# Renmusxd/PyIsingMonteCarlo

Hardware: AMD Instinct MI355X
Metric: spin-flip attempts/s (whole node), 4096^2 2D Ising (higher is better)
Workload: dtype u32; 1 GPU; c2: 4096x4096 periodic Ising J=-1 beta=0.4407, 256 replicas/GPU, checkerboard Metropolis, bit-packed spins, Philox4x32-10; replicas_per_gpu=256, parallelism=replicas x1

## Files before the change

pyisingmontecarlo_amd/csrc/lattice_kernels.hpp:

```cpp
#pragma once
#include "lattice_types.hpp"
#include "philox.hpp"
#include <type_traits>

namespace isingmc {

__device__ __forceinline__ uint32_t sel4(uint4 v, uint32_t i)
{
    return i == 0 ? v.x : i == 1 ? v.y : i == 2 ? v.z : v.w;
}

struct QuadNbr {
    uint32_t up[4], dn[4], ce[4], si[4];
};

template <bool UNI>
__device__ __forceinline__ void thread_to_quad(const LatGeom &g, uint32_t gid, uint32_t &Q, uint32_t &y,
                                               uint32_t &xw)
{
    if constexpr (UNI) {
        const uint32_t cl = uint32_t(g.cols_log2), col = gid & ((1u << cl) - 1);
        if (cl >= 6) {
            y = gid >> cl;
        } else {
// ... 75 lines not shown
        const uint32_t sw = mem.oth1(row_base(y) + sx);
        own[0] = o4.x; own[1] = o4.y; own[2] = o4.z; own[3] = o4.w;
        n.ce[0] = c4.x; n.ce[1] = c4.y; n.ce[2] = c4.z; n.ce[3] = c4.w;
        n.up[0] = u4.x; n.up[1] = u4.y; n.up[2] = u4.z; n.up[3] = u4.w;
        n.dn[0] = d4.x; n.dn[1] = d4.y; n.dn[2] = d4.z; n.dn[3] = d4.w;
        n.si[0] = sw;
        side_words(n, odd);
#pragma unroll
        for (int q = 0; q < 4; q++) widx[q] = w0 + q;
    } else {
#pragma unroll
        for (int q = 0; q < 4; q++) {
            const uint32_t w = 4 * Q + q;
            const uint32_t yy = w / g.wpr, xx = w - yy * g.wpr;
            const uint32_t yu = (yy == 0 ? g.H : yy) - 1, yd = (yy + 1 == g.H) ? 0 : yy + 1;
            const uint32_t row = yy * g.wpr;
            widx[q] = w;
            own[q] = mem.own1(w);
            n.ce[q] = mem.oth1(w);
            n.up[q] = mem.oth1(yu * g.wpr + xx);
            n.dn[q] = mem.oth1(yd * g.wpr + xx);
            if ((yy + colour) & 1) {
                const uint32_t nxt = mem.oth1(row + (xx + 1 == g.wpr ? 0 : xx + 1));
                n.si[q] = (n.ce[q] >> 1) | (nxt << 31);
            } else {
                const uint32_t prv = mem.oth1(row + (xx == 0 ? g.wpr : xx) - 1);
                n.si[q] = (n.ce[q] << 1) | (prv >> 31);
            }
        }
    }
}

template <bool PMJ>
__device__ __forceinline__ void bond_masks(const uint32_t own, const QuadNbr &n, int q,
                                           const uint32_t *__restrict__ jneg, uint32_t wpp,
                                           uint32_t widx, uint32_t jneg_uniform, uint32_t &a0,
                                           uint32_t &a1, uint32_t &a2, uint32_t &a3)
{
    if constexpr (PMJ) {
        a0 = own ^ n.up[q] ^ jneg[widx];
        a1 = own ^ n.dn[q] ^ jneg[wpp + widx];
        a2 = own ^ n.ce[q] ^ jneg[2 * wpp + widx];
        a3 = own ^ n.si[q] ^ jneg[3 * wpp + widx];
    } else {
        const uint32_t o = own ^ jneg_uniform;
        a0 = o ^ n.up[q];
        a1 = o ^ n.dn[q];
        a2 = o ^ n.ce[q];
        a3 = o ^ n.si[q];
    }
}

struct QuadState {
    uint32_t eq3[4], eq4[4], lt[4], und[4];
};

struct ThrBits {
    uint32_t hi3, hi4;
    uint32_t lo3, lo4;
    bool all3, all4;
    bool any_all;
};

__device__ __forceinline__ ThrBits thr_bits(const LatThr thr)
{
    ThrBits b;
    const uint32_t h3 = __builtin_amdgcn_readfirstlane(uint32_t(thr.T3 >> 32));
    const uint32_t h4 = __builtin_amdgcn_readfirstlane(uint32_t(thr.T4 >> 32));
    b.all3 = (h3 >> N_PLANES) != 0;
    b.all4 = (h4 >> N_PLANES) != 0;
    b.any_all = ((h3 | h4) >> N_PLANES) != 0;
    b.hi3 = h3 & ((1u << N_PLANES) - 1);
    b.hi4 = h4 & ((1u << N_PLANES) - 1);
    b.lo3 = uint32_t(thr.T3);
    b.lo4 = uint32_t(thr.T4);
    return b;
}

struct QuadSigns {
    uint32_t w[4][4];
};

template <bool PMJ>
__device__ __forceinline__ void load_signs(const uint32_t *__restrict__ jn, const LatGeom &g, const uint32_t Q, QuadSigns &js)
{
    if constexpr (PMJ) {
#pragma unroll
        for (int d = 0; d < 4; d++) {
            const uint4 v = *reinterpret_cast<const uint4 *>(jn + size_t(d) * g.wpp + 4 * size_t(Q));
            js.w[0][d] = v.x; js.w[1][d] = v.y; js.w[2][d] = v.z; js.w[3][d] = v.w;
        }
    }
}

__device__ __forceinline__ void class_masks(const uint32_t s01, const uint32_t c01, const uint32_t s23, const uint32_t c23,
                                            uint32_t &eq3, uint32_t &eq4)
{
    eq4 = c01 & c23;
    eq3 = __builtin_amdgcn_bitop3_b32(c01, s23, c23 & s01, 0xEA);
    asm("" : "+v"(eq3), "+v"(eq4));
}

template <bool PMJ>
__device__ __forceinline__ void quad_classes(const uint32_t own[4], const QuadNbr &n, const ThrBits &tb, const QuadSigns &js,
                                             const uint32_t jneg_uniform, QuadState &st)
{
    if constexpr (PMJ) {
#pragma unroll
        for (int q = 0; q < 4; q++) {
            const uint32_t a0 = own[q] ^ n.up[q] ^ js.w[q][0];
            const uint32_t a1 = own[q] ^ n.dn[q] ^ js.w[q][1];
            const uint32_t a2 = own[q] ^ n.ce[q] ^ js.w[q][2];
            const uint32_t a3 = own[q] ^ n.si[q] ^ js.w[q][3];
            class_masks(a0 ^ a1, a0 & a1, a2 ^ a3, a2 & a3, st.eq3[q], st.eq4[q]);
        }
    } else {
        uint32_t c01[4], c23[4];
        if (jneg_uniform) {
#pragma unroll
            for (int q = 0; q < 4; q++) {
                c01[q] = __builtin_amdgcn_bitop3_b32(own[q], n.up[q], n.dn[q], 0x81);
                c23[q] = __builtin_amdgcn_bitop3_b32(own[q], n.ce[q], n.si[q], 0x81);
            }
        } else {
#pragma unroll
            for (int q = 0; q < 4; q++) {
                c01[q] = __builtin_amdgcn_bitop3_b32(own[q], n.up[q], n.dn[q], 0x18);
                c23[q] = __builtin_amdgcn_bitop3_b32(own[q], n.ce[q], n.si[q], 0x18);
            }
        }
#pragma unroll
        for (int q = 0; q < 4; q++) class_masks(n.up[q] ^ n.dn[q], c01[q], n.ce[q] ^ n.si[q], c23[q], st.eq3[q], st.eq4[q]);
    }
    if (tb.any_all) {
#pragma unroll
        for (int q = 0; q < 4; q++) {
            if (tb.all3) st.eq3[q] = 0;
            if (tb.all4) st.eq4[q] = 0;
        }
    }
#pragma unroll
    for (int q = 0; q < 4; q++) {
        st.lt[q] = 0;
        st.und[q] = st.eq3[q] | st.eq4[q];
    }
}

__device__ __forceinline__ void plane_step(QuadState &st, const uint32_t rr[4], const int p, const ThrBits &tb)
{
    const auto step = [&](int q, uint32_t tbw) {
        st.lt[q] = __builtin_amdgcn_bitop3_b32(rr[q], tbw, st.lt[q], 0x8E);
        st.und[q] = __builtin_amdgcn_bitop3_b32(st.und[q], rr[q], tbw, 0x90);
    };
    const uint32_t sel = __builtin_amdgcn_readfirstlane(((tb.hi3 >> (N_PLANES - 1 - p)) & 1u) | (((tb.hi4 >> (N_PLANES - 1 - p)) & 1u) << 1));
    if (sel == 3) {
#pragma unroll
        for (int q = 0; q < 4; q++) step(q, st.eq3[q] | st.eq4[q]);
    } else if (sel == 1) {
#pragma unroll
        for (int q = 0; q < 4; q++) step(q, st.eq3[q]);
    } else if (sel == 2) {
#pragma unroll
        for (int q = 0; q < 4; q++) step(q, st.eq4[q]);
    } else {
#pragma unroll
        for (int q = 0; q < 4; q++) {
            st.lt[q] &= ~rr[q];
            st.und[q] &= ~rr[q];
        }
    }
}

template <int NQ>
__device__ __forceinline__ void quad_planes(QuadState (&st)[NQ], const uint32_t (&Q)[NQ], const uint32_t colour, const uint64_t t,
                                            const uint2 key, const PhiloxVKeys &vk, const ThrBits &tb)
{
    const uint32_t c0 = uint32_t(t);
#pragma unroll
    for (int p = N_PLANES - 1; p >= 0; p--) {
        uint32_t rr[NQ][4];
#pragma unroll
        for (int j = 0; j < NQ; j++) {
            const uint4 rnd = philox4x32_10(make_uint4(c0, Q[j], DOM_LAT_SWEEP, ctr2(t, colour, p)), key, vk);
            rr[j][0] = rnd.x; rr[j][1] = rnd.y; rr[j][2] = rnd.z; rr[j][3] = rnd.w;
        }
        auto step = [&](int j, int q, uint32_t tbw) {
            st[j].lt[q] = __builtin_amdgcn_bitop3_b32(rr[j][q], tbw, st[j].lt[q], 0x8E);
            st[j].und[q] = __builtin_amdgcn_bitop3_b32(st[j].und[q], rr[j][q], tbw, 0x90);
        };
        const uint32_t sel = __builtin_amdgcn_readfirstlane(((tb.hi3 >> (N_PLANES - 1 - p)) & 1u) | (((tb.hi4 >> (N_PLANES - 1 - p)) & 1u) << 1));
        if (sel == 3) {
#pragma unroll
            for (int j = 0; j < NQ; j++)
#pragma unroll
                for (int q = 0; q < 4; q++) step(j, q, st[j].eq3[q] | st[j].eq4[q]);
        } else if (sel == 1) {
#pragma unroll
            for (int j = 0; j < NQ; j++)
#pragma unroll
                for (int q = 0; q < 4; q++) step(j, q, st[j].eq3[q]);
        } else if (sel == 2) {
#pragma unroll
            for (int j = 0; j < NQ; j++)
#pragma unroll
                for (int q = 0; q < 4; q++) step(j, q, st[j].eq4[q]);
        } else {
#pragma unroll
            for (int j = 0; j < NQ; j++)
#pragma unroll
                for (int q = 0; q < 4; q++) {
                    st[j].lt[q] &= ~rr[j][q];
                    st[j].und[q] &= ~rr[j][q];
                }
        }
    }
}

struct QuadRandom {
    uint32_t rr[N_PLANES][4];
    uint4 tie;
};

__device__ __forceinline__ void quad_random(QuadRandom &R, const uint32_t Q, const uint32_t colour, const uint64_t t, const uint2 key,
                                            const PhiloxVKeys &vk)
{
    const uint32_t c0 = uint32_t(t);
#pragma unroll
    for (int p = 0; p < N_PLANES; p++) {
        const uint4 rnd = philox4x32_10(make_uint4(c0, Q, DOM_LAT_SWEEP, ctr2(t, colour, p)), key, vk);
        R.rr[p][0] = rnd.x; R.rr[p][1] = rnd.y; R.rr[p][2] = rnd.z; R.rr[p][3] = rnd.w;
    }
    R.tie = philox4x32_10(make_uint4(c0, Q, DOM_LAT_SWEEP, ctr2(t, colour, N_PLANES)), key, vk);
}

__device__ __forceinline__ void quad_ties(const QuadState &st, const uint32_t Q, const uint32_t colour, const uint64_t t,
                                          const uint2 key, const PhiloxVKeys &vk, const ThrBits &tb, uint32_t acc[4],
                                          const uint4 *first_call = nullptr)
{
    const uint32_t c0 = uint32_t(t), c1 = Q;
#pragma unroll
    for (int q = 0; q < 4; q++) acc[q] = __builtin_amdgcn_bitop3_b32(st.eq3[q], st.eq4[q], st.lt[q], 0xAB);
#ifdef ISINGMC_TIMING_ONLY_NO_TIES
    if (false) {
#else
    if (st.und[0] | st.und[1] | st.und[2] | st.und[3]) {
#endif
        const uint4 rnd = first_call ? *first_call : philox4x32_10(make_uint4(c0, c1, DOM_LAT_SWEEP, ctr2(t, colour, N_PLANES)), key, vk);
#ifdef ISINGMC_TIMING_ONLY_NO_TIE_LOOPS
        {
            const uint32_t rr4[4] = {rnd.x, rnd.y, rnd.z, rnd.w};
#pragma unroll
            for (int q = 0; q < 4; q++) acc[q] |= st.und[q] & (0u - uint32_t(rr4[q] < ((st.und[q] & st.eq4[q]) ? tb.lo4 : tb.lo3)));
            return;
        }
#endif
        const uint32_t n_ties = __popc(st.und[0]) + __popc(st.und[1]) + __popc(st.und[2]) + __popc(st.und[3]);
        if (n_ties <= 4) {
            uint32_t r0 = rnd.x, r1 = rnd.y, r2 = rnd.z, r3 = rnd.w;
            uint32_t lo3v, lo4v;
            asm volatile("v_mov_b32 %0, %1" : "=v"(lo3v) : "s"(tb.lo3));
            asm volatile("v_mov_b32 %0, %1" : "=v"(lo4v) : "s"(tb.lo4));
#pragma unroll
            for (int q = 0; q < 4; q++) {
                uint32_t m = st.und[q];
                while (m) {
                    const uint32_t bit = m & (0u - m);
                    m ^= bit;
                    const uint32_t lo = (bit & st.eq4[q]) ? lo4v : lo3v;
                    if (r0 < lo) acc[q] |= bit;
                    r0 = r1; r1 = r2; r2 = r3;
                }
            }
        } else {
            uint32_t nres = 0;
            uint4 w = rnd;
#pragma unroll
            for (int q = 0; q < 4; q++) {
                uint32_t m = st.und[q];
                while (m) {
                    const uint32_t b = __ffs(m) - 1;
                    m &= m - 1;
                    if (nres != 0 && (nres & 3u) == 0)
                        w = philox4x32_10(make_uint4(c0, c1, DOM_LAT_SWEEP, ctr2(t, colour, N_PLANES + (nres >> 2))), key, vk);
                    const uint32_t lo = ((st.eq4[q] >> b) & 1u) ? tb.lo4 : tb.lo3;
                    if (sel4(w, nres & 3u) < lo) acc[q] |= 1u << b;
                    nres++;
                }
            }
        }
    }
}

template <bool PMJ>
__device__ __forceinline__ void quad_flips(const uint32_t own[4], const QuadNbr &n, const uint32_t colour, const uint64_t t,
                                           const uint2 key, const PhiloxVKeys &vk,
                                           const LatThr thr, const QuadSigns &js, const uint32_t jneg_uniform,
                                           const uint32_t Q, uint32_t acc[4])
{
    const ThrBits tb = thr_bits(thr);
    QuadState st[1];
    const uint32_t Qs[1] = {Q};
    quad_classes<PMJ>(own, n, tb, js, jneg_uniform, st[0]);
    quad_planes<1>(st, Qs, colour, t, key, vk, tb);
    quad_ties(st[0], Q, colour, t, key, vk, tb, acc);
}

template <bool PMJ>
__device__ __forceinline__ void quad_flips_pre(const uint32_t own[4], const QuadNbr &n, const uint32_t colour, const uint64_t t,
                                               const uint2 key, const PhiloxVKeys &vk,
                                               const LatThr thr, const QuadSigns &js, const uint32_t jneg_uniform, const uint32_t Q,
                                               const QuadRandom &R, uint32_t acc[4])
{
    const ThrBits tb = thr_bits(thr);
    QuadState st;
    quad_classes<PMJ>(own, n, tb, js, jneg_uniform, st);
#pragma unroll
    for (int p = N_PLANES - 1; p >= 0; p--) plane_step(st, R.rr[p], p, tb);
    quad_ties(st, Q, colour, t, key, vk, tb, acc, &R.tie);
}

__device__ __forceinline__ void load_quad_uni(const BufPlanes &mem, const LatGeom &g, const uint32_t colour, const uint32_t gid,
                                              uint32_t &Q, uint32_t &vQ, uint32_t own[4], QuadNbr &n)
{
    typedef uint32_t u32x4 __attribute__((ext_vector_type(4)));
    const uint32_t cl = uint32_t(g.cols_log2), rb = 16u << cl;
    const uint32_t wave = __builtin_amdgcn_readfirstlane(gid >> 6), lane = gid & 63u;
    uint32_t y, col;
    bool lo_row, hi_row;
    uint32_t ypar;
    if (cl >= 6) {
        const uint32_t ys = wave >> (cl - 6);
        y = ys;
        col = gid & ((1u << cl) - 1);
        lo_row = ys == 0;
        hi_row = ys + 1 == g.H;
        ypar = ys & 1u;
    } else {
        const uint32_t rpw = 64u >> cl, ybase = ((wave >> 1) << (7 - cl)) + (wave & 1u);
        y = ybase + 2 * (lane >> cl);
        col = lane & ((1u << cl) - 1);
        lo_row = ybase == 0;
        hi_row = ybase + 2 * (rpw - 1) + 1 >= g.H;
        ypar = wave & 1u;
    }
    Q = (y << cl) + col;
    vQ = Q << 4;
    uint32_t vU, vD;
    if (lo_row | hi_row) {
        const uint32_t yu = (y == 0 ? g.H : y) - 1, yd = (y + 1 == g.H) ? 0 : y + 1;
        vU = ((yu << cl) + col) << 4;
        vD = ((yd << cl) + col) << 4;
    } else {
        vU = vQ - rb;
        vD = vQ + rb;
    }
    const bool odd = ((ypar + colour) & 1u) != 0;
    const uint32_t t16 = vQ & (rb - 1), rowb = vQ - t16;
    const uint32_t vS = rowb + (odd ? ((t16 + 16) & (rb - 1)) : ((t16 - 4) & (rb - 1)));
    const u32x4 o4 = __builtin_amdgcn_raw_buffer_load_b128(mem.rsrc, vQ, mem.own_off, 0);
    const u32x4 c4 = __builtin_amdgcn_raw_buffer_load_b128(mem.rsrc, vQ, mem.oth_off, 0);
    const u32x4 u4 = __builtin_amdgcn_raw_buffer_load_b128(mem.rsrc, vU, mem.oth_off, 0);
    const u32x4 d4 = __builtin_amdgcn_raw_buffer_load_b128(mem.rsrc, vD, mem.oth_off, 0);
    const uint32_t sw = __builtin_amdgcn_raw_buffer_load_b32(mem.rsrc, vS, mem.oth_off, 0);
    own[0] = o4.x; own[1] = o4.y; own[2] = o4.z; own[3] = o4.w;
    n.ce[0] = c4.x; n.ce[1] = c4.y; n.ce[2] = c4.z; n.ce[3] = c4.w;
    n.up[0] = u4.x; n.up[1] = u4.y; n.up[2] = u4.z; n.up[3] = u4.w;
    n.dn[0] = d4.x; n.dn[1] = d4.y; n.dn[2] = d4.z; n.dn[3] = d4.w;
    n.si[0] = sw;
    side_words(n, odd);
}

template <bool PMJ>
__device__ __forceinline__ void quad_measure(const uint32_t own_new[4], const QuadNbr &n, const QuadSigns &js,
                                             const uint32_t jneg_uniform, uint32_t &sat, uint32_t &up)
{
#pragma unroll
    for (int q = 0; q < 4; q++) {
        uint32_t a0, a1, a2, a3;
        if constexpr (PMJ) {
            a0 = own_new[q] ^ n.up[q] ^ js.w[q][0];
            a1 = own_new[q] ^ n.dn[q] ^ js.w[q][1];
            a2 = own_new[q] ^ n.ce[q] ^ js.w[q][2];
            a3 = own_new[q] ^ n.si[q] ^ js.w[q][3];
        } else {
            const uint32_t o = own_new[q] ^ jneg_uniform;
            a0 = o ^ n.up[q]; a1 = o ^ n.dn[q]; a2 = o ^ n.ce[q]; a3 = o ^ n.si[q];
        }
        sat += __popc(a0) + __popc(a1) + __popc(a2) + __popc(a3);
        (void)up;
    }
}

struct PendingQuad {
    uint32_t w[4];
    uint32_t widx[4];
};

template <bool VEC, typename Mem>
__device__ __forceinline__ void store_pending(const Mem &mem, const PendingQuad &p)
{
    if constexpr (VEC) {
        mem.store4(p.widx[0], make_uint4(p.w[0], p.w[1], p.w[2], p.w[3]));
    } else {
#pragma unroll
        for (int q = 0; q < 4; q++) mem.store1(p.widx[q], p.w[q]);
    }
}

template <bool VEC, bool PMJ, bool UNI, typename Mem, bool MEASURE = false>
__device__ __forceinline__ void update_quad(const Mem &mem, const LatGeom &g, const uint32_t colour, const uint64_t t, const uint2 key,
                                            const PhiloxVKeys &vk, const LatThr thr, const uint32_t *__restrict__ jn,
                                            const uint32_t jneg_uniform, const uint32_t gid, uint32_t *sat = nullptr,
                                            uint32_t *up = nullptr, PendingQuad *pending = nullptr)
{
    if constexpr (VEC && UNI && std::is_same<Mem, BufPlanes>::value) {
        typedef uint32_t u32x4 __attribute__((ext_vector_type(4)));
        uint32_t Q, vQ, own[4], acc[4];
        QuadNbr n;
        QuadSigns js;
        load_quad_uni(mem, g, colour, gid, Q, vQ, own, n);
        load_signs<PMJ>(jn, g, Q, js);
        quad_flips<PMJ>(own, n, colour, t, key, vk, thr, js, jneg_uniform, Q, acc);
        if constexpr (MEASURE) {
#pragma unroll
            for (int q = 0; q < 4; q++) { pending->w[q] = own[q] ^ acc[q]; pending->widx[q] = 4 * Q + q; }
            quad_measure<PMJ>(pending->w, n, js, jneg_uniform, *sat, *up);
        } else {
            __builtin_amdgcn_raw_buffer_store_b128(u32x4{own[0] ^ acc[0], own[1] ^ acc[1], own[2] ^ acc[2], own[3] ^ acc[3]}, mem.rsrc,
                                                   vQ, mem.own_off, 0);
        }
        return;
    }
    uint32_t Q, qy, qxw;
    thread_to_quad<UNI>(g, gid, Q, qy, qxw);

    uint32_t own[4], widx[4], acc[4];
    QuadNbr n;
    QuadSigns js;
    load_signs<PMJ>(jn, g, Q, js);
    load_quad<VEC, UNI>(mem, g, colour, Q, qy, qxw, own, n, widx);
    quad_flips<PMJ>(own, n, colour, t, key, vk, thr, js, jneg_uniform, Q, acc);

    if constexpr (MEASURE) {
#pragma unroll
        for (int q = 0; q < 4; q++) { pending->w[q] = own[q] ^ acc[q]; pending->widx[q] = widx[q]; }
        quad_measure<PMJ>(pending->w, n, js, jneg_uniform, *sat, *up);
    } else if constexpr (VEC) {
        mem.store4(widx[0], make_uint4(own[0] ^ acc[0], own[1] ^ acc[1], own[2] ^ acc[2], own[3] ^ acc[3]));
    } else {
#pragma unroll
        for (int q = 0; q < 4; q++) mem.store1(widx[q], own[q] ^ acc[q]);
    }
}

constexpr uint32_t MEASURE_SLOTS = 16;
#ifndef ISINGMC_MEASURE_WAVES
#define ISINGMC_MEASURE_WAVES 7
#endif

template <bool VEC, bool PMJ, bool UNI>
__global__ __launch_bounds__(256, ISINGMC_MEASURE_WAVES) void lat_sweep_measure_kernel(
    uint32_t *__restrict__ state, const LatGeom g, const uint64_t t, const uint2 *__restrict__ keys, const LatThr thr_uniform,
    const LatThr *__restrict__ thr_replica, const uint32_t *__restrict__ jneg, const uint32_t jneg_uniform,
    unsigned long long *__restrict__ out, const size_t out_stride)
{
    __shared__ uint32_t red[2][4];
    const uint32_t colour = 1;
    const uint32_t r = blockIdx.y;
    const uint32_t gid = blockIdx.x * 256 + threadIdx.x;
    uint32_t sat = 0, up = 0;
    BufPlanes mem;
    mem.rsrc = __builtin_amdgcn_make_buffer_rsrc(state + size_t(r) * 2 * g.wpp, 0, int(2 * g.wpp * sizeof(uint32_t)), 0x00020000);
    mem.own_off = colour * g.wpp * 4u;
    mem.oth_off = 0;
    PendingQuad pending;
    if (gid < g.nquads) {
        const uint2 key = keys[r];
        update_quad<VEC, PMJ, UNI, BufPlanes, true>(mem, g, colour, t, key, philox_vkeys(key), thr_replica ? thr_replica[r] : thr_uniform,
                                                    PMJ ? jneg + size_t(colour) * 4 * g.wpp : nullptr, jneg_uniform, gid, &sat, &up, &pending);
    }
#pragma unroll
    for (int off = 32; off > 0; off >>= 1) sat += __shfl_xor(sat, off);
    if ((threadIdx.x & 63) == 0) red[0][threadIdx.x >> 6] = sat;
    __syncthreads();
    if (threadIdx.x == 0) {
        unsigned long long *slot = out + size_t(r) * out_stride + 2 * (blockIdx.x % MEASURE_SLOTS);
        atomicAdd(slot, (unsigned long long)(red[0][0] + red[0][1] + red[0][2] + red[0][3]));
    }
    if (gid < g.nquads) store_pending<VEC>(mem, pending);
}

template <bool VEC, bool PMJ, bool UNI>
__global__ __launch_bounds__(256) void lat_sweep_kernel(
    uint32_t *__restrict__ state, const LatGeom g, const uint32_t colour, const uint64_t t,
    const uint2 *__restrict__ keys, const LatThr thr_uniform, const LatThr *__restrict__ thr_replica,
    const uint32_t *__restrict__ jneg, const uint32_t jneg_uniform)
{
    const uint32_t r = blockIdx.y;
    const uint32_t gid = blockIdx.x * 256 + threadIdx.x;
    if (gid >= g.nquads) return;
    BufPlanes mem;
    mem.rsrc = __builtin_amdgcn_make_buffer_rsrc(state + size_t(r) * 2 * g.wpp, 0, int(2 * g.wpp * sizeof(uint32_t)), 0x00020000);
    mem.own_off = colour * g.wpp * 4u;
    mem.oth_off = (1 - colour) * g.wpp * 4u;
// ... 12 lines not shown
    const uint32_t r = blockIdx.y;
    const uint32_t stride = gridDim.x * 256;
    const uint32_t gid = blockIdx.x * 256 + threadIdx.x;
    BufPlanes mem;
    mem.rsrc = __builtin_amdgcn_make_buffer_rsrc(state + size_t(r) * 2 * g.wpp, 0, int(2 * g.wpp * sizeof(uint32_t)), 0x00020000);
    mem.own_off = colour * g.wpp * 4u;
    mem.oth_off = (1 - colour) * g.wpp * 4u;
    const uint2 key = keys[r];
    const PhiloxVKeys vk = philox_vkeys(key);
    const ThrBits tb = thr_bits(thr_replica ? thr_replica[r] : thr_uniform);
    const uint32_t *jn = PMJ ? jneg + size_t(colour) * 4 * g.wpp : nullptr;

    const uint32_t cl = uint32_t(g.cols_log2), rb = 16u << cl;
    const uint32_t wave = __builtin_amdgcn_readfirstlane(gid >> 6), lane = gid & 63u;
    uint32_t ys, span;
    uint32_t Q;
    bool odd;
    if (cl >= 6) {
        ys = wave >> (cl - 6);
        span = 1;
        Q = gid;
        odd = ((ys + colour) & 1u) != 0;
    } else {
        const uint32_t rpw = 64u >> cl;
        ys = ((wave >> 1) << (7 - cl)) + (wave & 1u);
        span = 2 * (rpw - 1) + 1;
        Q = ((ys + 2 * (lane >> cl)) << cl) + (lane & ((1u << cl) - 1));
        odd = ((wave + colour) & 1u) != 0;
    }
    const uint32_t vQ = Q << 4, t16 = vQ & (rb - 1);
    const uint32_t vS = (vQ - t16) + (odd ? ((t16 + 16) & (rb - 1)) : ((t16 - 4) & (rb - 1)));
    const uint32_t row_step = stride >> cl, byte_step = stride << 4;
    const bool from_row0 = ys == 0;
    uint32_t walked = 0;
#pragma unroll 1
    for (uint32_t it = 0; it < iters; it++) {
        uint32_t vU, vD, s_ud;
        if (from_row0 | (ys + span >= g.H)) {
            const uint32_t y = Q >> cl, col = Q & ((1u << cl) - 1);
            const uint32_t yu = (y == 0 ? g.H : y) - 1, yd = (y + 1 == g.H) ? 0 : y + 1;
            vU = ((yu << cl) + col) << 4;
            vD = ((yd << cl) + col) << 4;
            s_ud = mem.oth_off;
        } else {
            vU = vQ - rb;
            vD = vQ + rb;
            s_ud = mem.oth_off + walked;
        }
        const u32x4 o4 = __builtin_amdgcn_raw_buffer_load_b128(mem.rsrc, vQ, mem.own_off + walked, 0);
        const u32x4 c4 = __builtin_amdgcn_raw_buffer_load_b128(mem.rsrc, vQ, mem.oth_off + walked, 0);
        const u32x4 u4 = __builtin_amdgcn_raw_buffer_load_b128(mem.rsrc, vU, s_ud, 0);
        const u32x4 d4 = __builtin_amdgcn_raw_buffer_load_b128(mem.rsrc, vD, s_ud, 0);
        const uint32_t sw = __builtin_amdgcn_raw_buffer_load_b32(mem.rsrc, vS, mem.oth_off + walked, 0);
        uint32_t own[4] = {o4.x, o4.y, o4.z, o4.w}, acc[4];
        QuadNbr n;
        n.ce[0] = c4.x; n.ce[1] = c4.y; n.ce[2] = c4.z; n.ce[3] = c4.w;
        n.up[0] = u4.x; n.up[1] = u4.y; n.up[2] = u4.z; n.up[3] = u4.w;
        n.dn[0] = d4.x; n.dn[1] = d4.y; n.dn[2] = d4.z; n.dn[3] = d4.w;
        n.si[0] = sw;
        side_words(n, odd);
        QuadSigns js;
        load_signs<PMJ>(jn, g, Q, js);
        QuadState st[1];
        const uint32_t Qs[1] = {Q};
        quad_classes<PMJ>(own, n, tb, js, jneg_uniform, st[0]);
        quad_planes<1>(st, Qs, colour, t, key, vk, tb);
        quad_ties(st[0], Q, colour, t, key, vk, tb, acc);
        __builtin_amdgcn_raw_buffer_store_b128(u32x4{own[0] ^ acc[0], own[1] ^ acc[1], own[2] ^ acc[2], own[3] ^ acc[3]}, mem.rsrc, vQ,
                                               mem.own_off + walked, 0);
        Q += stride;
        ys += row_step;
        walked += byte_step;
    }
}

__attribute__((unused)) static __global__ __launch_bounds__(256) void lat_init_kernel(uint32_t *__restrict__ state, const LatGeom g,
                                                       const uint2 *__restrict__ keys,
                                                       const uint32_t first_replica)
{
    const uint32_t r = first_replica + blockIdx.y;
    const uint32_t Q = blockIdx.x * 256 + threadIdx.x;
    if (Q >= 2 * g.nquads) return;
    const uint32_t c = Q >= g.nquads, q = Q - c * g.nquads;
    const uint4 rnd = philox4x32_10(make_uint4(0, q, ctr2(0, c, 0), DOM_LAT_INIT), keys[r]);
    *reinterpret_cast<uint4 *>(state + size_t(r) * 2 * g.wpp + size_t(c) * g.wpp + 4 * size_t(q)) = rnd;
}

constexpr uint32_t MEASURE_QUADS_PER_THREAD = 16;

template <bool VEC, bool PMJ>
__global__ __launch_bounds__(256) void lat_measure_kernel(
    const uint32_t *__restrict__ state, const LatGeom g, const uint32_t *__restrict__ jneg,
    const uint32_t jneg_uniform, unsigned long long *__restrict__ out, const size_t out_stride)
{
    __shared__ uint32_t red[2][4];
    const uint32_t r = blockIdx.y;
    uint32_t sat = 0, up = 0;
    const uint32_t *p0 = state + size_t(r) * 2 * g.wpp;
    for (uint32_t i = 0; i < MEASURE_QUADS_PER_THREAD; i++) {
        const uint32_t gid = (blockIdx.x * MEASURE_QUADS_PER_THREAD + i) * 256 + threadIdx.x;
        if (gid >= g.nquads) break;
        uint32_t Q, qy, qxw, own[4], widx[4];
        thread_to_quad<false>(g, gid, Q, qy, qxw);
        QuadNbr n;
        load_quad<VEC, false>(PtrPlanes{const_cast<uint32_t *>(p0), p0 + g.wpp}, g, 0, Q, qy, qxw, own, n, widx);
#pragma unroll
        for (int q = 0; q < 4; q++) {
            uint32_t a0, a1, a2, a3;
            bond_masks<PMJ>(own[q], n, q, jneg, g.wpp, widx[q], jneg_uniform, a0, a1, a2, a3);
            sat += __popc(a0) + __popc(a1) + __popc(a2) + __popc(a3);
            up += __popc(own[q]) + __popc(n.ce[q]);
        }
    }
#pragma unroll
    for (int off = 32; off > 0; off >>= 1) {
        sat += __shfl_xor(sat, off);
        up += __shfl_xor(up, off);
    }
    if ((threadIdx.x & 63) == 0) {
        red[0][threadIdx.x >> 6] = sat;
        red[1][threadIdx.x >> 6] = up;
    }
// ... 82 lines not shown
```

pyisingmontecarlo_amd/csrc/spread_kernels.hpp:

```cpp
#pragma once
#include "lattice_kernels.hpp"
#include "spread_types.hpp"

namespace isingmc {

static_assert(N_PLANES == 7, "lat_resident_spread_kernel: eight lanes per quad = 7 bit planes + the first residual call");
template <bool VEC, bool PMJ, int LPQ>
__global__ __launch_bounds__(1024) void lat_resident_spread_kernel(
    uint32_t *__restrict__ state, const LatGeom g, const uint64_t t0, const uint32_t timesteps,
    const uint2 *__restrict__ keys, const LatThr *__restrict__ thr_steps, const uint32_t thr_stride,
    const LatThr *__restrict__ thr_replica, const uint32_t *__restrict__ jneg, const uint32_t jneg_uniform,
    unsigned long long *__restrict__ steps_out, const uint32_t n_replicas)
{
    extern __shared__ __attribute__((aligned(16))) uint32_t planes[];
    __shared__ uint32_t red[2][16];
    const uint32_t r = blockIdx.x, tid = threadIdx.x, nthreads = blockDim.x;
    uint4 *s_rand = reinterpret_cast<uint4 *>(planes + 2 * g.wpp);
    uint32_t *mine = state + size_t(r) * 2 * g.wpp;
    for (uint32_t i = tid; i < g.wpp / 2; i += nthreads)
        reinterpret_cast<uint4 *>(planes)[i] = reinterpret_cast<const uint4 *>(mine)[i];
    const uint2 key = keys[r];
    const PhiloxVKeys vk = philox_vkeys(key);
    const uint32_t quad = tid / LPQ, call = tid % LPQ;
    __syncthreads();
    for (uint32_t k = 0; k < timesteps; k++) {
        const LatThr thr = thr_replica ? thr_replica[r] : thr_steps[size_t(k) * thr_stride];
        const uint64_t t = t0 + k;
        for (uint32_t colour = 0; colour < 2; colour++) {
            if (quad < g.nquads) {
#pragma unroll
                for (uint32_t c = 0; c < 8 / LPQ; c++)
                    s_rand[8 * quad + call + LPQ * c] = philox4x32_10(make_uint4(uint32_t(t), quad, DOM_LAT_SWEEP, ctr2(t, colour, call + LPQ * c)), key, vk);
            }
            __syncthreads();
            if (tid < g.nquads) {
                QuadRandom R;
#pragma unroll
                for (int p = 0; p < N_PLANES; p++) {
                    const uint4 v = s_rand[8 * tid + p];
                    R.rr[p][0] = v.x; R.rr[p][1] = v.y; R.rr[p][2] = v.z; R.rr[p][3] = v.w;
                }
                R.tie = s_rand[8 * tid + N_PLANES];
                const PtrPlanes mem{planes + colour * g.wpp, planes + (1 - colour) * g.wpp};
                uint32_t Q, qy, qxw, own[4], widx[4], acc[4];
                thread_to_quad<false>(g, tid, Q, qy, qxw);
                QuadNbr n;
                QuadSigns js;
                load_signs<PMJ>(PMJ ? jneg + size_t(colour) * 4 * g.wpp : nullptr, g, Q, js);
                load_quad<VEC, false>(mem, g, colour, Q, qy, qxw, own, n, widx);
                quad_flips_pre<PMJ>(own, n, colour, t, key, vk, thr, js, jneg_uniform, Q, R, acc);
                if constexpr (VEC) {
                    mem.store4(widx[0], make_uint4(own[0] ^ acc[0], own[1] ^ acc[1], own[2] ^ acc[2], own[3] ^ acc[3]));
                } else {
#pragma unroll
                    for (int q = 0; q < 4; q++) mem.store1(widx[q], own[q] ^ acc[q]);
                }
            }
            __syncthreads();
        }
        if (steps_out) {
            uint32_t sat = 0, up = 0;
            for (uint32_t gid = tid; gid < g.nquads; gid += nthreads) {
                uint32_t Q, qy, qxw, own[4], widx[4];
                thread_to_quad<false>(g, gid, Q, qy, qxw);
                QuadNbr n;
                load_quad<VEC, false>(PtrPlanes{planes, planes + g.wpp}, g, 0, Q, qy, qxw, own, n, widx);
#pragma unroll
                for (int q = 0; q < 4; q++) {
                    uint32_t a0, a1, a2, a3;
                    bond_masks<PMJ>(own[q], n, q, jneg, g.wpp, widx[q], jneg_uniform, a0, a1, a2, a3);
                    sat += __popc(a0) + __popc(a1) + __popc(a2) + __popc(a3);
                    up += __popc(own[q]) + __popc(n.ce[q]);
                }
            }
#pragma unroll
            for (int off = 32; off > 0; off >>= 1) {
                sat += __shfl_xor(sat, off);
                up += __shfl_xor(up, off);
            }
            if ((tid & 63) == 0) { red[0][tid >> 6] = sat; red[1][tid >> 6] = up; }
            __syncthreads();
            if (tid == 0) {
                unsigned long long sum = 0, u = 0;
                for (uint32_t w = 0; w < (nthreads + 63) / 64; w++) { sum += red[0][w]; u += red[1][w]; }
                steps_out[(size_t(k) * n_replicas + r) * 2] = sum;
                steps_out[(size_t(k) * n_replicas + r) * 2 + 1] = u;
            }
            __syncthreads();
        }
    }
    for (uint32_t i = tid; i < g.wpp / 2; i += nthreads)
        reinterpret_cast<uint4 *>(mine)[i] = reinterpret_cast<const uint4 *>(planes)[i];
}

}
```

pyisingmontecarlo_amd/csrc/strip_kernels.hpp:

```cpp
#pragma once
#include "lattice_kernels.hpp"
#include "strip_types.hpp"

namespace isingmc {

__device__ __forceinline__ double strip_det_exp(double x)
{
    if (x >= 0.0) return 1.0;
    if (x < -40.0) return 0.0;
    const double LOG2E = 1.4426950408889634074;
    const double LN2_HI = 6.93147180369123816490e-01, LN2_LO = 1.90821492927058770002e-10;
    const double kf = floor(fma(x, LOG2E, 0.5));
    double r = fma(-kf, LN2_HI, x);
    r = fma(-kf, LN2_LO, r);
    double p = 1.0 / 6227020800.0;
    p = fma(p, r, 1.0 / 479001600.0);
    p = fma(p, r, 1.0 / 39916800.0);
    p = fma(p, r, 1.0 / 3628800.0);
    p = fma(p, r, 1.0 / 362880.0);
    p = fma(p, r, 1.0 / 40320.0);
    p = fma(p, r, 1.0 / 5040.0);
    p = fma(p, r, 1.0 / 720.0);
    p = fma(p, r, 1.0 / 120.0);
    p = fma(p, r, 1.0 / 24.0);
    p = fma(p, r, 1.0 / 6.0);
    p = fma(p, r, 0.5);
    p = fma(p, r, 1.0);
    p = fma(p, r, 1.0);
    const long long k = (long long)kf;
    return p * __longlong_as_double((1023ll + k) << 52);
}

__device__ __forceinline__ bool strip_wait_granule(const unsigned long long *p, const uint32_t want, uint32_t &value, uint32_t *err)
{
    const unsigned long long start = __builtin_amdgcn_s_memrealtime();
    uint32_t spins = 0;
    for (;;) {
        const unsigned long long v = __hip_atomic_load((strip_gu64)p, __ATOMIC_RELAXED, __HIP_MEMORY_SCOPE_AGENT);
        if (uint32_t(v >> 32) == want) {
            value = uint32_t(v);
            return true;
        }
        __builtin_amdgcn_s_sleep(1);
        if ((++spins & 63u) == 0 && (__builtin_amdgcn_s_memrealtime() - start > STRIP_TIMEOUT_TICKS ||
                                     __hip_atomic_load((strip_gu32)err, __ATOMIC_RELAXED, __HIP_MEMORY_SCOPE_AGENT) != 0)) {
            atomicOr(err, STRIP_ERR_TIMEOUT);
            return false;
        }
    }
}

__device__ __forceinline__ size_t strip_granule(const LatGeom &g, uint32_t strip, uint32_t plane, uint32_t side)
{
    return ((size_t(strip) * 2 + plane) * 2 + side) * g.wpr;
}

template <bool PMJ>
__device__ __forceinline__ void strip_update_quad(uint32_t *lds, const uint32_t PL, const LatGeom &g, const uint32_t colour,
                                                  const uint32_t yl, const uint32_t col, const uint32_t Q, const bool odd, const uint64_t t,
                                                  const uint2 key, const PhiloxVKeys &vk, const LatThr thr,
                                                  const uint32_t *__restrict__ jn, const uint32_t jneg_uniform, const QuadRandom &R,
                                                  uint32_t new_words[4], const bool measure, uint32_t &sat, uint32_t &up)
{
    const uint32_t wpr = g.wpr, xw = 4 * col;
    uint32_t *ownp = lds + colour * PL;
    const uint32_t *othp = lds + (1 - colour) * PL;
    const uint32_t w0 = yl * wpr + xw;
    QuadSigns js;
    load_signs<PMJ>(jn, g, Q, js);
    const uint4 o4 = *reinterpret_cast<const uint4 *>(ownp + w0);
    const uint4 c4 = *reinterpret_cast<const uint4 *>(othp + w0);
    const uint4 u4 = *reinterpret_cast<const uint4 *>(othp + w0 - wpr);
    const uint4 d4 = *reinterpret_cast<const uint4 *>(othp + w0 + wpr);
    const uint32_t sx = odd ? (xw + 4 == wpr ? 0 : xw + 4) : (xw == 0 ? wpr : xw) - 1;
    QuadNbr n;
    n.si[0] = othp[yl * wpr + sx];
    uint32_t own[4] = {o4.x, o4.y, o4.z, o4.w}, acc[4];
    n.ce[0] = c4.x; n.ce[1] = c4.y; n.ce[2] = c4.z; n.ce[3] = c4.w;
    n.up[0] = u4.x; n.up[1] = u4.y; n.up[2] = u4.z; n.up[3] = u4.w;
    n.dn[0] = d4.x; n.dn[1] = d4.y; n.dn[2] = d4.z; n.dn[3] = d4.w;
    side_words(n, odd);
#ifdef ISINGMC_STRIP_NO_PRECOMPUTE
    (void)R;
    quad_flips<PMJ>(own, n, colour, t, key, vk, thr, js, jneg_uniform, Q, acc);
#else
    quad_flips_pre<PMJ>(own, n, colour, t, key, vk, thr, js, jneg_uniform, Q, R, acc);
#endif
#pragma unroll
    for (int q = 0; q < 4; q++) new_words[q] = own[q] ^ acc[q];
    *reinterpret_cast<uint4 *>(ownp + w0) = make_uint4(new_words[0], new_words[1], new_words[2], new_words[3]);
    if (measure) quad_measure<PMJ>(new_words, n, js, jneg_uniform, sat, up);
}

template <bool PMJ, int NW, bool LAD>
__global__ __launch_bounds__(64 * NW, 4) void lat_strip_kernel(
    uint32_t *__restrict__ state, const LatGeom g, const StripArgs a, const uint64_t t0, const uint32_t timesteps,
    const uint2 *__restrict__ keys, const LatThr *__restrict__ thr_steps, const uint32_t thr_stride,
    const LatThr *__restrict__ thr_replica, const uint32_t *__restrict__ jneg, const uint32_t jneg_uniform,
    unsigned long long *__restrict__ halo, unsigned long long *__restrict__ steps_out, const StripFinal fin, const StripLadder lad,
    const uint32_t n_replicas, uint32_t *__restrict__ err)
{
    constexpr uint32_t NT = 64 * NW;
    extern __shared__ __attribute__((aligned(16))) uint32_t lds[];
    const uint32_t tid = threadIdx.x, wpr = g.wpr, S = a.S;
    const uint32_t PL = (S + 2) * wpr;
    uint32_t *red = lds + 2 * PL;
    uint32_t r, strip;
    if (a.xcd_remap) {
        const uint32_t x = blockIdx.x & 7u, m = blockIdx.x >> 3;
        strip = m % a.n_strips;
        r = x + 8 * (m / a.n_strips);
    } else {
        r = blockIdx.x / a.n_strips;
        strip = blockIdx.x - r * a.n_strips;
    }
    const uint32_t y0 = strip * S;
    const uint32_t up_strip = strip == 0 ? a.n_strips - 1 : strip - 1, dn_strip = strip + 1 == a.n_strips ? 0 : strip + 1;
    uint32_t *mine = state + size_t(r) * 2 * g.wpp;
    unsigned long long *rep_halo = halo + size_t(r) * a.n_strips * 4 * wpr;

#pragma unroll
    for (uint32_t p = 0; p < 2; p++)
        reinterpret_cast<uint4 *>(lds + p * PL + wpr)[tid] = reinterpret_cast<const uint4 *>(mine + size_t(p) * g.wpp + size_t(y0) * wpr)[tid];
    const uint32_t y_up = (y0 == 0 ? g.H : y0) - 1, y_dn = (y0 + S == g.H) ? 0 : y0 + S;
    for (uint32_t i = tid; i < 4 * wpr; i += NT) {
        const uint32_t p = i / (2 * wpr), side = (i / wpr) & 1u, w = i % wpr;
        lds[p * PL + (side ? (S + 1) * wpr : 0) + w] = mine[size_t(p) * g.wpp + size_t(side ? y_dn : y_up) * wpr + w];
    }
    if (NW > 1 && tid == 0) red[8] = 0;
    uint32_t my_rung = 0;
    if constexpr (LAD) {
        if (tid == 0) red[9] = 0;
        if constexpr (NW > 1) __syncthreads();
        for (uint32_t i = tid; i < lad.n_rungs; i += NT)
            if (lad.perm_in[i] == r) red[9] = i;
        if constexpr (NW > 1) __syncthreads();
        my_rung = __builtin_amdgcn_readfirstlane(red[9]);
    }
    const uint2 key = keys[r];
    const PhiloxVKeys vk = philox_vkeys(key);

    const uint32_t ql = a.qpr_log2, wave = tid >> 6, lane = tid & 63u;
// ... 187 lines not shown
```

Before: 11230 billion spin-flip attempts/s.

## Merge zero threshold-bit plane pairs and fold flip mask into single bitop3

Drops the eq3 class mask from per-quad state and replaces it with und0 (eq3|eq4); sel==1 plane steps now use a negated eq4 bitop3 variant. Consecutive zero threshold planes are merged into one bitop3 that combines the previous and current random words, halving the update work on those planes. The final own^acc flip is folded into one bitop3 over own, und0 and lt, and ties write into lt directly. The intent is to cut VALU instructions and register pressure in the Metropolis comparison chain, at the cost of more complex plane-selection logic that must stay uniform across the wavefront.

```diff
diff --git a/pyisingmontecarlo_amd/csrc/lattice_kernels.hpp b/pyisingmontecarlo_amd/csrc/lattice_kernels.hpp
--- a/pyisingmontecarlo_amd/csrc/lattice_kernels.hpp
+++ b/pyisingmontecarlo_amd/csrc/lattice_kernels.hpp
@@ -151,7 +151,7 @@
 }
 
 struct QuadState {
-    uint32_t eq3[4], eq4[4], lt[4], und[4];
+    uint32_t eq4[4], lt[4], und[4], und0[4];
 };
 
 struct ThrBits {
@@ -204,6 +204,7 @@
 __device__ __forceinline__ void quad_classes(const uint32_t own[4], const QuadNbr &n, const ThrBits &tb, const QuadSigns &js,
                                              const uint32_t jneg_uniform, QuadState &st)
 {
+    uint32_t eq3[4];
     if constexpr (PMJ) {
 #pragma unroll
         for (int q = 0; q < 4; q++) {
@@ -211,7 +212,7 @@
             const uint32_t a1 = own[q] ^ n.dn[q] ^ js.w[q][1];
             const uint32_t a2 = own[q] ^ n.ce[q] ^ js.w[q][2];
             const uint32_t a3 = own[q] ^ n.si[q] ^ js.w[q][3];
-            class_masks(a0 ^ a1, a0 & a1, a2 ^ a3, a2 & a3, st.eq3[q], st.eq4[q]);
+            class_masks(a0 ^ a1, a0 & a1, a2 ^ a3, a2 & a3, eq3[q], st.eq4[q]);
         }
     } else {
         uint32_t c01[4], c23[4];
@@ -229,52 +230,92 @@
             }
         }
 #pragma unroll
-        for (int q = 0; q < 4; q++) class_masks(n.up[q] ^ n.dn[q], c01[q], n.ce[q] ^ n.si[q], c23[q], st.eq3[q], st.eq4[q]);
+        for (int q = 0; q < 4; q++) class_masks(n.up[q] ^ n.dn[q], c01[q], n.ce[q] ^ n.si[q], c23[q], eq3[q], st.eq4[q]);
     }
     if (tb.any_all) {
 #pragma unroll
         for (int q = 0; q < 4; q++) {
-            if (tb.all3) st.eq3[q] = 0;
+            if (tb.all3) eq3[q] = 0;
             if (tb.all4) st.eq4[q] = 0;
         }
     }
 #pragma unroll
     for (int q = 0; q < 4; q++) {
         st.lt[q] = 0;
-        st.und[q] = st.eq3[q] | st.eq4[q];
-    }
-}
-
-__device__ __forceinline__ void plane_step(QuadState &st, const uint32_t rr[4], const int p, const ThrBits &tb)
+        st.und0[q] = eq3[q] | st.eq4[q];
+        st.und[q] = st.und0[q];
+    }
+}
+
+constexpr uint32_t BITOP_FLIP = 0x4B;
+__device__ __forceinline__ void quad_new_words(const uint32_t own[4], const QuadState &st, uint32_t neww[4])
+{
+#pragma unroll
+    for (int q = 0; q < 4; q++) neww[q] = __builtin_amdgcn_bitop3_b32(own[q], st.und0[q], st.lt[q], BITOP_FLIP);
+}
+
+constexpr uint32_t BITOP_ZERO_PAIR = 0x10;
+constexpr uint32_t BITOP_LT = 0x8E, BITOP_UND = 0x90, BITOP_LT_NOT = 0x2B, BITOP_UND_NOT = 0x60;
+constexpr uint32_t SEL_ZERO_PAIR = 4, SEL_ZERO_OPEN = 5;
+
+constexpr bool PLANE_MERGE = true;
+
+template <bool MERGE>
+__device__ __forceinline__ uint32_t plane_selector(const ThrBits &tb, const int p, const bool open)
+{
+    const uint32_t i = N_PLANES - 1 - p;
+    uint32_t sel = ((tb.hi3 >> i) & 1u) | (((tb.hi4 >> i) & 1u) << 1);
+    if constexpr (MERGE) {
+        if (open) sel = SEL_ZERO_PAIR;
+        else if (sel == 0 && p > 0 && (((tb.hi3 | tb.hi4) >> (i + 1)) & 1u) == 0) sel = SEL_ZERO_OPEN;
+    }
+    return __builtin_amdgcn_readfirstlane(sel);
+}
+
+__device__ __forceinline__ bool plane_step(QuadState &st, const uint32_t rr[4], const uint32_t prev[4], const int p, const ThrBits &tb,
+                                           const bool open)
 {
     const auto step = [&](int q, uint32_t tbw) {
-        st.lt[q] = __builtin_amdgcn_bitop3_b32(rr[q], tbw, st.lt[q], 0x8E);
-        st.und[q] = __builtin_amdgcn_bitop3_b32(st.und[q], rr[q], tbw, 0x90);
+        st.lt[q] = __builtin_amdgcn_bitop3_b32(rr[q], tbw, st.lt[q], BITOP_LT);
+        st.und[q] = __builtin_amdgcn_bitop3_b32(st.und[q], rr[q], tbw, BITOP_UND);
     };
-    const uint32_t sel = __builtin_amdgcn_readfirstlane(((tb.hi3 >> (N_PLANES - 1 - p)) & 1u) | (((tb.hi4 >> (N_PLANES - 1 - p)) & 1u) << 1));
+    const auto step_not = [&](int q, uint32_t ntbw) {
+        st.lt[q] = __builtin_amdgcn_bitop3_b32(rr[q], ntbw, st.lt[q], BITOP_LT_NOT);
+        st.und[q] = __builtin_amdgcn_bitop3_b32(st.und[q], rr[q], ntbw, BITOP_UND_NOT);
+    };
+    const uint32_t sel = plane_selector<PLANE_MERGE>(tb, p, open);
     if (sel == 3) {
 #pragma unroll
-        for (int q = 0; q < 4; q++) step(q, st.eq3[q] | st.eq4[q]);
+        for (int q = 0; q < 4; q++) step(q, st.und0[q]);
     } else if (sel == 1) {
 #pragma unroll
-        for (int q = 0; q < 4; q++) step(q, st.eq3[q]);
+        for (int q = 0; q < 4; q++) step_not(q, st.eq4[q]);
     } else if (sel == 2) {
 #pragma unroll
         for (int q = 0; q < 4; q++) step(q, st.eq4[q]);
-    } else {
+    } else if (PLANE_MERGE && sel == SEL_ZERO_PAIR) {
+#pragma unroll
+        for (int q = 0; q < 4; q++) {
+            st.lt[q] = __builtin_amdgcn_bitop3_b32(st.lt[q], prev[q], rr[q], BITOP_ZERO_PAIR);
+            st.und[q] = __builtin_amdgcn_bitop3_b32(st.und[q], prev[q], rr[q], BITOP_ZERO_PAIR);
+        }
+    } else if (sel == 0) {
 #pragma unroll
         for (int q = 0; q < 4; q++) {
             st.lt[q] &= ~rr[q];
             st.und[q] &= ~rr[q];
         }
     }
-}
-
-template <int NQ>
+    return PLANE_MERGE && sel == SEL_ZERO_OPEN;
+}
+
+template <int NQ, bool MERGE = PLANE_MERGE>
 __device__ __forceinline__ void quad_planes(QuadState (&st)[NQ], const uint32_t (&Q)[NQ], const uint32_t colour, const uint64_t t,
                                             const uint2 key, const PhiloxVKeys &vk, const ThrBits &tb)
 {
     const uint32_t c0 = uint32_t(t);
+    uint32_t prev[NQ][4];
+    bool open = false;
 #pragma unroll
     for (int p = N_PLANES - 1; p >= 0; p--) {
         uint32_t rr[NQ][4];
@@ -284,26 +325,38 @@
             rr[j][0] = rnd.x; rr[j][1] = rnd.y; rr[j][2] = rnd.z; rr[j][3] = rnd.w;
         }
         auto step = [&](int j, int q, uint32_t tbw) {
-            st[j].lt[q] = __builtin_amdgcn_bitop3_b32(rr[j][q], tbw, st[j].lt[q], 0x8E);
-            st[j].und[q] = __builtin_amdgcn_bitop3_b32(st[j].und[q], rr[j][q], tbw, 0x90);
+            st[j].lt[q] = __builtin_amdgcn_bitop3_b32(rr[j][q], tbw, st[j].lt[q], BITOP_LT);
+            st[j].und[q] = __builtin_amdgcn_bitop3_b32(st[j].und[q], rr[j][q], tbw, BITOP_UND);
         };
-        const uint32_t sel = __builtin_amdgcn_readfirstlane(((tb.hi3 >> (N_PLANES - 1 - p)) & 1u) | (((tb.hi4 >> (N_PLANES - 1 - p)) & 1u) << 1));
+        auto step_not = [&](int j, int q, uint32_t ntbw) {
+            st[j].lt[q] = __builtin_amdgcn_bitop3_b32(rr[j][q], ntbw, st[j].lt[q], BITOP_LT_NOT);
+            st[j].und[q] = __builtin_amdgcn_bitop3_b32(st[j].und[q], rr[j][q], ntbw, BITOP_UND_NOT);
+        };
+        const uint32_t sel = plane_selector<MERGE>(tb, p, open);
         if (sel == 3) {
 #pragma unroll
             for (int j = 0; j < NQ; j++)
 #pragma unroll
-                for (int q = 0; q < 4; q++) step(j, q, st[j].eq3[q] | st[j].eq4[q]);
+                for (int q = 0; q < 4; q++) step(j, q, st[j].und0[q]);
         } else if (sel == 1) {
 #pragma unroll
             for (int j = 0; j < NQ; j++)
 #pragma unroll
-                for (int q = 0; q < 4; q++) step(j, q, st[j].eq3[q]);
+                for (int q = 0; q < 4; q++) step_not(j, q, st[j].eq4[q]);
         } else if (sel == 2) {
 #pragma unroll
             for (int j = 0; j < NQ; j++)
 #pragma unroll
                 for (int q = 0; q < 4; q++) step(j, q, st[j].eq4[q]);
-        } else {
+        } else if (MERGE && p < N_PLANES - 1 && sel == SEL_ZERO_PAIR) {
+#pragma unroll
+            for (int j = 0; j < NQ; j++)
+#pragma unroll
+                for (int q = 0; q < 4; q++) {
+                    st[j].lt[q] = __builtin_amdgcn_bitop3_b32(st[j].lt[q], prev[j][q], rr[j][q], BITOP_ZERO_PAIR);
+                    st[j].und[q] = __builtin_amdgcn_bitop3_b32(st[j].und[q], prev[j][q], rr[j][q], BITOP_ZERO_PAIR);
+                }
+        } else if (sel == 0) {
 #pragma unroll
             for (int j = 0; j < NQ; j++)
 #pragma unroll
@@ -311,7 +364,17 @@
                     st[j].lt[q] &= ~rr[j][q];
                     st[j].und[q] &= ~rr[j][q];
                 }
-        }
+        } else if (MERGE) {
+#pragma unroll
+            for (int j = 0; j < NQ; j++)
+#pragma unroll
+                for (int q = 0; q < 4; q++) asm volatile("" : "+v"(st[j].lt[q]), "+v"(st[j].und[q]));
+        }
+        open = MERGE && sel == SEL_ZERO_OPEN;
+#pragma unroll
+        for (int j = 0; j < NQ; j++)
+#pragma unroll
+            for (int q = 0; q < 4; q++) prev[j][q] = rr[j][q];
     }
 }
 
@@ -332,13 +395,11 @@
     R.tie = philox4x32_10(make_uint4(c0, Q, DOM_LAT_SWEEP, ctr2(t, colour, N_PLANES)), key, vk);
 }
 
-__device__ __forceinline__ void quad_ties(const QuadState &st, const uint32_t Q, const uint32_t colour, const uint64_t t,
-                                          const uint2 key, const PhiloxVKeys &vk, const ThrBits &tb, uint32_t acc[4],
+__device__ __forceinline__ void quad_ties(QuadState &st, const uint32_t Q, const uint32_t colour, const uint64_t t,
+                                          const uint2 key, const PhiloxVKeys &vk, const ThrBits &tb,
                                           const uint4 *first_call = nullptr)
 {
     const uint32_t c0 = uint32_t(t), c1 = Q;
-#pragma unroll
-    for (int q = 0; q < 4; q++) acc[q] = __builtin_amdgcn_bitop3_b32(st.eq3[q], st.eq4[q], st.lt[q], 0xAB);
 #ifdef ISINGMC_TIMING_ONLY_NO_TIES
     if (false) {
 #else
@@ -349,7 +410,7 @@
         {
             const uint32_t rr4[4] = {rnd.x, rnd.y, rnd.z, rnd.w};
 #pragma unroll
-            for (int q = 0; q < 4; q++) acc[q] |= st.und[q] & (0u - uint32_t(rr4[q] < ((st.und[q] & st.eq4[q]) ? tb.lo4 : tb.lo3)));
+            for (int q = 0; q < 4; q++) st.lt[q] |= st.und[q] & (0u - uint32_t(rr4[q] < ((st.und[q] & st.eq4[q]) ? tb.lo4 : tb.lo3)));
             return;
         }
 #endif
@@ -366,7 +427,7 @@
                     const uint32_t bit = m & (0u - m);
                     m ^= bit;
                     const uint32_t lo = (bit & st.eq4[q]) ? lo4v : lo3v;
-                    if (r0 < lo) acc[q] |= bit;
+                    if (r0 < lo) st.lt[q] |= bit;
                     r0 = r1; r1 = r2; r2 = r3;
                 }
             }
@@ -382,7 +443,7 @@
                     if (nres != 0 && (nres & 3u) == 0)
                         w = philox4x32_10(make_uint4(c0, c1, DOM_LAT_SWEEP, ctr2(t, colour, N_PLANES + (nres >> 2))), key, vk);
                     const uint32_t lo = ((st.eq4[q] >> b) & 1u) ? tb.lo4 : tb.lo3;
-                    if (sel4(w, nres & 3u) < lo) acc[q] |= 1u << b;
+                    if (sel4(w, nres & 3u) < lo) st.lt[q] |= 1u << b;
                     nres++;
                 }
             }
@@ -390,32 +451,35 @@
     }
 }
 
-template <bool PMJ>
+template <bool PMJ, bool MERGE = PLANE_MERGE>
 __device__ __forceinline__ void quad_flips(const uint32_t own[4], const QuadNbr &n, const uint32_t colour, const uint64_t t,
                                            const uint2 key, const PhiloxVKeys &vk,
                                            const LatThr thr, const QuadSigns &js, const uint32_t jneg_uniform,
-                                           const uint32_t Q, uint32_t acc[4])
+                                           const uint32_t Q, uint32_t neww[4])
 {
     const ThrBits tb = thr_bits(thr);
     QuadState st[1];
     const uint32_t Qs[1] = {Q};
     quad_classes<PMJ>(own, n, tb, js, jneg_uniform, st[0]);
-    quad_planes<1>(st, Qs, colour, t, key, vk, tb);
-    quad_ties(st[0], Q, colour, t, key, vk, tb, acc);
+    quad_planes<1, MERGE>(st, Qs, colour, t, key, vk, tb);
+    quad_ties(st[0], Q, colour, t, key, vk, tb);
+    quad_new_words(own, st[0], neww);
 }
 
 template <bool PMJ>
 __device__ __forceinline__ void quad_flips_pre(const uint32_t own[4], const QuadNbr &n, const uint32_t colour, const uint64_t t,
                                                const uint2 key, const PhiloxVKeys &vk,
                                                const LatThr thr, const QuadSigns &js, const uint32_t jneg_uniform, const uint32_t Q,
-                                               const QuadRandom &R, uint32_t acc[4])
+                                               const QuadRandom &R, uint32_t neww[4])
 {
     const ThrBits tb = thr_bits(thr);
     QuadState st;
     quad_classes<PMJ>(own, n, tb, js, jneg_uniform, st);
-#pragma unroll
-    for (int p = N_PLANES - 1; p >= 0; p--) plane_step(st, R.rr[p], p, tb);
-    quad_ties(st, Q, colour, t, key, vk, tb, acc, &R.tie);
+    bool open = false;
+#pragma unroll
+    for (int p = N_PLANES - 1; p >= 0; p--) open = plane_step(st, R.rr[p], R.rr[p < N_PLANES - 1 ? p + 1 : p], p, tb, open);
+    quad_ties(st, Q, colour, t, key, vk, tb, &R.tie);
+    quad_new_words(own, st, neww);
 }
 
 __device__ __forceinline__ void load_quad_uni(const BufPlanes &mem, const LatGeom &g, const uint32_t colour, const uint32_t gid,
@@ -514,41 +578,40 @@
 {
     if constexpr (VEC && UNI && std::is_same<Mem, BufPlanes>::value) {
         typedef uint32_t u32x4 __attribute__((ext_vector_type(4)));
-        uint32_t Q, vQ, own[4], acc[4];
+        uint32_t Q, vQ, own[4], neww[4];
         QuadNbr n;
         QuadSigns js;
         load_quad_uni(mem, g, colour, gid, Q, vQ, own, n);
         load_signs<PMJ>(jn, g, Q, js);
-        quad_flips<PMJ>(own, n, colour, t, key, vk, thr, js, jneg_uniform, Q, acc);
+        quad_flips<PMJ, PLANE_MERGE && !MEASURE>(own, n, colour, t, key, vk, thr, js, jneg_uniform, Q, neww);
         if constexpr (MEASURE) {
 #pragma unroll
-            for (int q = 0; q < 4; q++) { pending->w[q] = own[q] ^ acc[q]; pending->widx[q] = 4 * Q + q; }
+            for (int q = 0; q < 4; q++) { pending->w[q] = neww[q]; pending->widx[q] = 4 * Q + q; }
             quad_measure<PMJ>(pending->w, n, js, jneg_uniform, *sat, *up);
         } else {
-            __builtin_amdgcn_raw_buffer_store_b128(u32x4{own[0] ^ acc[0], own[1] ^ acc[1], own[2] ^ acc[2], own[3] ^ acc[3]}, mem.rsrc,
-                                                   vQ, mem.own_off, 0);
+            __builtin_amdgcn_raw_buffer_store_b128(u32x4{neww[0], neww[1], neww[2], neww[3]}, mem.rsrc, vQ, mem.own_off, 0);
         }
         return;
     }
     uint32_t Q, qy, qxw;
     thread_to_quad<UNI>(g, gid, Q, qy, qxw);
 
-    uint32_t own[4], widx[4], acc[4];
+    uint32_t own[4], widx[4], neww[4];
     QuadNbr n;
     QuadSigns js;
     load_signs<PMJ>(jn, g, Q, js);
     load_quad<VEC, UNI>(mem, g, colour, Q, qy, qxw, own, n, widx);
-    quad_flips<PMJ>(own, n, colour, t, key, vk, thr, js, jneg_uniform, Q, acc);
+    quad_flips<PMJ, PLANE_MERGE && !MEASURE>(own, n, colour, t, key, vk, thr, js, jneg_uniform, Q, neww);
 
     if constexpr (MEASURE) {
 #pragma unroll
-        for (int q = 0; q < 4; q++) { pending->w[q] = own[q] ^ acc[q]; pending->widx[q] = widx[q]; }
+        for (int q = 0; q < 4; q++) { pending->w[q] = neww[q]; pending->widx[q] = widx[q]; }
         quad_measure<PMJ>(pending->w, n, js, jneg_uniform, *sat, *up);
     } else if constexpr (VEC) {
-        mem.store4(widx[0], make_uint4(own[0] ^ acc[0], own[1] ^ acc[1], own[2] ^ acc[2], own[3] ^ acc[3]));
-    } else {
-#pragma unroll
-        for (int q = 0; q < 4; q++) mem.store1(widx[q], own[q] ^ acc[q]);
+        mem.store4(widx[0], make_uint4(neww[0], neww[1], neww[2], neww[3]));
+    } else {
+#pragma unroll
+        for (int q = 0; q < 4; q++) mem.store1(widx[q], neww[q]);
     }
 }
 
@@ -667,7 +730,7 @@
         const u32x4 u4 = __builtin_amdgcn_raw_buffer_load_b128(mem.rsrc, vU, s_ud, 0);
         const u32x4 d4 = __builtin_amdgcn_raw_buffer_load_b128(mem.rsrc, vD, s_ud, 0);
         const uint32_t sw = __builtin_amdgcn_raw_buffer_load_b32(mem.rsrc, vS, mem.oth_off + walked, 0);
-        uint32_t own[4] = {o4.x, o4.y, o4.z, o4.w}, acc[4];
+        uint32_t own[4] = {o4.x, o4.y, o4.z, o4.w}, neww[4];
         QuadNbr n;
         n.ce[0] = c4.x; n.ce[1] = c4.y; n.ce[2] = c4.z; n.ce[3] = c4.w;
         n.up[0] = u4.x; n.up[1] = u4.y; n.up[2] = u4.z; n.up[3] = u4.w;
@@ -680,9 +743,9 @@
         const uint32_t Qs[1] = {Q};
         quad_classes<PMJ>(own, n, tb, js, jneg_uniform, st[0]);
         quad_planes<1>(st, Qs, colour, t, key, vk, tb);
-        quad_ties(st[0], Q, colour, t, key, vk, tb, acc);
-        __builtin_amdgcn_raw_buffer_store_b128(u32x4{own[0] ^ acc[0], own[1] ^ acc[1], own[2] ^ acc[2], own[3] ^ acc[3]}, mem.rsrc, vQ,
-                                               mem.own_off + walked, 0);
+        quad_ties(st[0], Q, colour, t, key, vk, tb);
+        quad_new_words(own, st[0], neww);
+        __builtin_amdgcn_raw_buffer_store_b128(u32x4{neww[0], neww[1], neww[2], neww[3]}, mem.rsrc, vQ, mem.own_off + walked, 0);
         Q += stride;
         ys += row_step;
         walked += byte_step;
diff --git a/pyisingmontecarlo_amd/csrc/spread_kernels.hpp b/pyisingmontecarlo_amd/csrc/spread_kernels.hpp
--- a/pyisingmontecarlo_amd/csrc/spread_kernels.hpp
+++ b/pyisingmontecarlo_amd/csrc/spread_kernels.hpp
@@ -42,18 +42,18 @@
                 }
                 R.tie = s_rand[8 * tid + N_PLANES];
                 const PtrPlanes mem{planes + colour * g.wpp, planes + (1 - colour) * g.wpp};
-                uint32_t Q, qy, qxw, own[4], widx[4], acc[4];
+                uint32_t Q, qy, qxw, own[4], widx[4], neww[4];
                 thread_to_quad<false>(g, tid, Q, qy, qxw);
                 QuadNbr n;
                 QuadSigns js;
                 load_signs<PMJ>(PMJ ? jneg + size_t(colour) * 4 * g.wpp : nullptr, g, Q, js);
                 load_quad<VEC, false>(mem, g, colour, Q, qy, qxw, own, n, widx);
-                quad_flips_pre<PMJ>(own, n, colour, t, key, vk, thr, js, jneg_uniform, Q, R, acc);
+                quad_flips_pre<PMJ>(own, n, colour, t, key, vk, thr, js, jneg_uniform, Q, R, neww);
                 if constexpr (VEC) {
-                    mem.store4(widx[0], make_uint4(own[0] ^ acc[0], own[1] ^ acc[1], own[2] ^ acc[2], own[3] ^ acc[3]));
+                    mem.store4(widx[0], make_uint4(neww[0], neww[1], neww[2], neww[3]));
                 } else {
 #pragma unroll
-                    for (int q = 0; q < 4; q++) mem.store1(widx[q], own[q] ^ acc[q]);
+                    for (int q = 0; q < 4; q++) mem.store1(widx[q], neww[q]);
                 }
             }
             __syncthreads();
diff --git a/pyisingmontecarlo_amd/csrc/strip_kernels.hpp b/pyisingmontecarlo_amd/csrc/strip_kernels.hpp
--- a/pyisingmontecarlo_amd/csrc/strip_kernels.hpp
+++ b/pyisingmontecarlo_amd/csrc/strip_kernels.hpp
@@ -75,19 +75,17 @@
     const uint32_t sx = odd ? (xw + 4 == wpr ? 0 : xw + 4) : (xw == 0 ? wpr : xw) - 1;
     QuadNbr n;
     n.si[0] = othp[yl * wpr + sx];
-    uint32_t own[4] = {o4.x, o4.y, o4.z, o4.w}, acc[4];
+    const uint32_t own[4] = {o4.x, o4.y, o4.z, o4.w};
     n.ce[0] = c4.x; n.ce[1] = c4.y; n.ce[2] = c4.z; n.ce[3] = c4.w;
     n.up[0] = u4.x; n.up[1] = u4.y; n.up[2] = u4.z; n.up[3] = u4.w;
     n.dn[0] = d4.x; n.dn[1] = d4.y; n.dn[2] = d4.z; n.dn[3] = d4.w;
     side_words(n, odd);
 #ifdef ISINGMC_STRIP_NO_PRECOMPUTE
     (void)R;
-    quad_flips<PMJ>(own, n, colour, t, key, vk, thr, js, jneg_uniform, Q, acc);
+    quad_flips<PMJ>(own, n, colour, t, key, vk, thr, js, jneg_uniform, Q, new_words);
 #else
-    quad_flips_pre<PMJ>(own, n, colour, t, key, vk, thr, js, jneg_uniform, Q, R, acc);
-#endif
-#pragma unroll
-    for (int q = 0; q < 4; q++) new_words[q] = own[q] ^ acc[q];
+    quad_flips_pre<PMJ>(own, n, colour, t, key, vk, thr, js, jneg_uniform, Q, R, new_words);
+#endif
     *reinterpret_cast<uint4 *>(ownp + w0) = make_uint4(new_words[0], new_words[1], new_words[2], new_words[3]);
     if (measure) quad_measure<PMJ>(new_words, n, js, jneg_uniform, sat, up);
 }
```

After: 11360 billion spin-flip attempts/s, median of 6. +1.1%, better.
